# JuliaSmoothOptimizers/CaNNOLeS.jl

Measured on AMD Instinct MI355X. Metric: Newton systems/sec (fp64), batched n=1e4 NLS; achieved HBM GB/s vs peak, higher is better.
Workload: dtype f64; 1 GPU; cfg3 band constrained NLS n=10000 nequ=10000 ncon=50, 16384 independent problems per GPU, one newton_system! per problem per step; batch_per_gpu=16384, total_problems=16384, ordering=canonical+early, nnzL_stored=145150, nnzL_exact=100180, fronts=1000, all_success=True

## Files before the change

cannoles.jl_amd/csrc/band.hip:

```cpp
#include <hip/hip_runtime.h>

#include "band.h"
#include "kernels.h"

namespace cnl {

namespace {

template <class T>
__device__ __forceinline__ T* as_global(T* p) {
  return (T*)(__attribute__((address_space(1))) T*)p;
}

typedef const __attribute__((address_space(4))) int* cptr;
__device__ __forceinline__ cptr as_const(const int* p) { return (cptr)(const __attribute__((address_space(1))) int*)p; }

constexpr int NPC = BAND_NPIECE;
constexpr int LANE_D = BAND_LANE_DOUBLES;
constexpr int EXCH_OFF = BAND_IN_OFF;
static_assert(48 <= BAND_NPIECE * 8, "exchange area inside the operand pieces");

__device__ __forceinline__ constexpr int sidx(int a, int b) { return a >= b ? a * (a + 1) / 2 + b : b * (b + 1) / 2 + a; }

template <class T>
__device__ __forceinline__ T rrcp(T d) {
  T r;
  if constexpr (sizeof(T) == 8) r = __builtin_amdgcn_rcp(d);
  else r = __builtin_amdgcn_rcpf(d);
  const T e = fma(-d, r, T(1));
  return fma(r, e, r);
}
template <class T>
__device__ __forceinline__ T rdiv(T w, T d, T r) {
  const T q = w * r;
  const T res = fma(-d, q, w);
  return fma(res, r, q);
}


constexpr int NS = BAND_NS;
template <class T>
struct Win {
  T S[NS * (NS + 1) / 2];
  T X[NS];
  T S55;
  T c[NS];
  T c5;
};
__device__ __forceinline__ constexpr int lslot(int PH, int k) { return (PH - BAND_HW + k + NS) % NS; }

#define LDSD(off) (*reinterpret_cast<const T*>(myb + (off)))
#define LDSW(off) (*reinterpret_cast<T*>(myb + (off)))

struct Rec { int v[BAND_SW]; };
struct RowRec { int v[BAND_RW]; };
__device__ __forceinline__ void load_rec(Rec& R, const char* recb, int o) {
  const int4* q = reinterpret_cast<const int4*>(recb + 4 * o);
#pragma unroll
  for (int k = 0; k < BAND_SW / 4; k++) { const int4 t = q[k]; R.v[4 * k] = t.x; R.v[4 * k + 1] = t.y; R.v[4 * k + 2] = t.z; R.v[4 * k + 3] = t.w; }
}
__device__ __forceinline__ void load_row(RowRec& R, const char* recb, int o) {
  const int4* q = reinterpret_cast<const int4*>(recb + 4 * o);
#pragma unroll
  for (int k = 0; k < BAND_RW / 4; k++) { const int4 t = q[k]; R.v[4 * k] = t.x; R.v[4 * k + 1] = t.y; R.v[4 * k + 2] = t.z; R.v[4 * k + 3] = t.w; }
}

template <class T>
struct FOps { T eo[15]; T rj[BAND_NB]; T rdr, rrr; };
template <class T>
__device__ __forceinline__ void fload(FOps<T>& P, const Rec& st, const RowRec& row0, const int fl, char* myb) {
#pragma unroll
  for (int q = 0; q < 15; q++) P.eo[q] = LDSD(st.v[BS_DG0 + q]);
  static_assert(BS_RX == BS_DG0 + 14, "the fifteen operands of an entering variable are consecutive words of the step block");
  P.rdr = T(1); P.rrr = T(0);
#pragma unroll
  for (int k = 0; k < BAND_NB; k++) P.rj[k] = T(0);
  if ((fl >> 8) & 255) {
#pragma unroll
    for (int k = 0; k < BAND_NB; k++) P.rj[k] = LDSD(row0.v[BR_J0 + k]);
    P.rdr = LDSD(row0.v[BR_DI]);
    P.rrr = LDSD(row0.v[BR_RR]);
  }
}

__device__ __forceinline__ long long band_il_offset(int e, int stride) { return stride ? (long long)(e >> 3) * stride + (e & 7) : (long long)e; }

template <int PH, class T>
__device__ __forceinline__ void fstep(Win<T>& W, const FOps<T>& OP, const Rec& st, const int fl, const char* recb, const int o, char* myb,
                                      const T* __restrict__ gvals, const T* __restrict__ grhs, cptr borders, long long pv, long long pr,
                                      bool has_rhs, T rho, bool ovr, T tol, int& npos, int& nzer, const int vstride = 0, const int rstride = 0) {
  constexpr int es = PH, ps = lslot(PH, 0);
  const int nrows = (fl >> 8) & 255;
  const T (&eo)[15] = OP.eo;
  const T (&rj)[BAND_NB] = OP.rj;
  const T rdr = OP.rdr, rrr = OP.rrr;
  {
    const T dg = (eo[0] + eo[1]) + eo[2];
    T rv = eo[BS_RHO - BS_DG0];
    if (!(fl & (1 << 16))) rv = ovr ? rho : rv;
    W.S[sidx(es, es)] = dg + rv;
#pragma unroll
    for (int k = 1; k <= BAND_HW; k++) W.S[sidx(es, lslot(PH, BAND_HW - k))] = eo[BS_OD - BS_DG0 + 2 * (k - 1)] + eo[BS_OD - BS_DG0 + 2 * (k - 1) + 1];
    W.X[es] = eo[BS_BC0 - BS_DG0] + eo[BS_BC1 - BS_DG0];
    W.c[es] = eo[BS_RX - BS_DG0];
  }
  for (int i = 0; i < nrows; i++) {
    T J[BAND_NB], dr, rr;
    if (i == 0) {
#pragma unroll
      for (int k = 0; k < BAND_NB; k++) J[k] = rj[k];
      dr = rdr; rr = rrr;
    } else {
      RowRec rb;
      load_row(rb, recb, o + BAND_SW + BAND_RW * i);
#pragma unroll
      for (int k = 0; k < BAND_NB; k++) J[k] = LDSD(rb.v[BR_J0 + k]);
      dr = LDSD(rb.v[BR_DI]);
      rr = LDSD(rb.v[BR_RR]);
    }
    npos += dr > tol;
    nzer += fabs(dr) <= tol;
    const T r = rrcp(dr);
    const T w = rdiv(T(-1), dr, r);
    const T tr = rr * w;
#pragma unroll
    for (int ka = 0; ka < BAND_NB; ka++) {
      const T ta = J[ka] * w;
#pragma unroll
      for (int kb = 0; kb <= ka; kb++) W.S[sidx(lslot(PH, ka), lslot(PH, kb))] = fma(ta, J[kb], W.S[sidx(lslot(PH, ka), lslot(PH, kb))]);
      W.c[lslot(PH, ka)] = fma(tr, J[ka], W.c[lslot(PH, ka)]);
    }
  }
  if (fl & BF_PIVOT_B) {
    cptr bt = borders + BAND_BW * __builtin_amdgcn_readfirstlane(st.v[BS_BORDER]);
    W.S55 += gvals[pv + band_il_offset(bt[BB_DSRC], vstride)];
    W.c5 += has_rhs ? grhs[pr + band_il_offset(bt[BB_RHS], rstride)] : T(0);
    const T d = W.S55;
    npos += d > tol;
    nzer += fabs(d) <= tol;
    const T r = rrcp(d);
    T l[BAND_NB], w[BAND_NB];
#pragma unroll
    for (int k = 0; k < BAND_NB; k++) { w[k] = W.X[lslot(PH, k)]; l[k] = rdiv(w[k], d, r); }
    const T z = rdiv(W.c5, d, r);
#pragma unroll
    for (int ka = 0; ka < BAND_NB; ka++) {
#pragma unroll
      for (int kb = 0; kb <= ka; kb++) W.S[sidx(lslot(PH, ka), lslot(PH, kb))] = fma(w[ka], -l[kb], W.S[sidx(lslot(PH, ka), lslot(PH, kb))]);
      W.c[lslot(PH, ka)] = fma(w[ka], -z, W.c[lslot(PH, ka)]);
    }
    T* lo = reinterpret_cast<T*>(myb + st.v[BS_LB]);
#pragma unroll
    for (int k = 0; k < BAND_NB; k++) lo[k] = l[k];
    lo[BAND_NB] = z;
#pragma unroll
    for (int k = 0; k < BAND_NB; k++) W.X[lslot(PH, k)] = T(0);
    W.S55 = T(0); W.c5 = T(0);
  }
  if (fl & BF_PIVOT_X) {
    const T d = W.S[sidx(ps, ps)];
    npos += d > tol;
    nzer += fabs(d) <= tol;
    const T r = rrcp(d);
    T l[BAND_NB], w[BAND_NB];
#pragma unroll
    for (int k = 1; k < BAND_NB; k++) { w[k] = W.S[sidx(lslot(PH, k), ps)]; l[k] = rdiv(w[k], d, r); }
    const T w5 = W.X[ps], l5 = rdiv(w5, d, r), z = rdiv(W.c[ps], d, r);
#pragma unroll
    for (int ka = 1; ka < BAND_NB; ka++) {
#pragma unroll
      for (int kb = 1; kb <= ka; kb++) W.S[sidx(lslot(PH, ka), lslot(PH, kb))] = fma(w[ka], -l[kb], W.S[sidx(lslot(PH, ka), lslot(PH, kb))]);
      W.X[lslot(PH, ka)] = fma(w5, -l[ka], W.X[lslot(PH, ka)]);
      W.c[lslot(PH, ka)] = fma(w[ka], -z, W.c[lslot(PH, ka)]);
    }
    W.S55 = fma(w5, -l5, W.S55);
    W.c5 = fma(w5, -z, W.c5);
    T* lo = reinterpret_cast<T*>(myb + st.v[BS_LX]);
#pragma unroll
    for (int k = 1; k < BAND_NB; k++) lo[k - 1] = l[k];
    lo[4] = l5;
    lo[5] = z;
  }
}

template <class T>
struct BOps { T lx[BAND_LREC], lb[BAND_LREC], rj[BAND_NB]; T rdr, rrr; };
template <class T>
__device__ __forceinline__ void bload(BOps<T>& P, const Rec& st, const RowRec& row0, const int fl, char* myb) {
#pragma unroll
  for (int q = 0; q < BAND_LREC; q++) { P.lx[q] = T(0); P.lb[q] = T(0); }
#pragma unroll
  for (int k = 0; k < BAND_NB; k++) P.rj[k] = T(0);
  P.rdr = T(1); P.rrr = T(0);
  if (fl & BF_PIVOT_X) {
    const T* lo = reinterpret_cast<const T*>(myb + st.v[BS_LX]);
#pragma unroll
    for (int q = 0; q < BAND_LREC; q++) P.lx[q] = lo[q];
  }
  if (fl & BF_PIVOT_B) {
    const T* lo = reinterpret_cast<const T*>(myb + st.v[BS_LB]);
#pragma unroll
    for (int q = 0; q < BAND_LREC; q++) P.lb[q] = lo[q];
  }
  if ((fl >> 8) & 255) {
#pragma unroll
    for (int k = 0; k < BAND_NB; k++) P.rj[k] = LDSD(row0.v[BR_J0 + k]);
    P.rdr = LDSD(row0.v[BR_DI]);
    P.rrr = LDSD(row0.v[BR_RR]);
  }
}
template <int PH, class T>
__device__ __forceinline__ void bstep(T (&xs)[NS + 1], const BOps<T>& OP, const Rec& st, const RowRec& row0, const int fl, const char* recb,
                                      const int o, char* myb, cptr borders, T* __restrict__ gd, long long pd, bool okme) {
  constexpr int ps = lslot(PH, 0);
  const int nrows = (fl >> 8) & 255;
  const T (&lx)[BAND_LREC] = OP.lx;
  const T (&lb)[BAND_LREC] = OP.lb;
  const T (&rj)[BAND_NB] = OP.rj;
  const T rdr = OP.rdr, rrr = OP.rrr;
  if (fl & BF_PIVOT_X) {
    T x = lx[5];
#pragma unroll
    for (int k = 1; k < BAND_NB; k++) x = fma(-lx[k - 1], xs[lslot(PH, k)], x);
    x = fma(-lx[4], xs[NS], x);
    xs[ps] = x;
    LDSW(st.v[BS_DX]) = -x;
  }
  if (fl & BF_PIVOT_B) {
    T x = lb[BAND_NB];
#pragma unroll
    for (int k = 0; k < BAND_NB; k++) x = fma(-lb[k], xs[lslot(PH, k)], x);
    xs[NS] = x;
    if (okme) gd[pd + borders[BAND_BW * __builtin_amdgcn_readfirstlane(st.v[BS_BORDER]) + BB_DOUT]] = -x;
  }
  for (int i = 0; i < nrows; i++) {
    T J[BAND_NB], dr, rr;
    int dro;
    if (i == 0) {
#pragma unroll
      for (int k = 0; k < BAND_NB; k++) J[k] = rj[k];
      dr = rdr; rr = rrr; dro = row0.v[BR_DR];
    } else {
      RowRec rb;
      load_row(rb, recb, o + BAND_SW + BAND_RW * i);
#pragma unroll
      for (int k = 0; k < BAND_NB; k++) J[k] = LDSD(rb.v[BR_J0 + k]);
      dr = LDSD(rb.v[BR_DI]); rr = LDSD(rb.v[BR_RR]); dro = rb.v[BR_DR];
    }
    T acc = -rr;
#pragma unroll
    for (int k = 0; k < BAND_NB; k++) acc = fma(J[k], xs[lslot(PH, k)], acc);
    LDSW(dro) = rdiv(acc, dr, rrcp(dr));
  }
  if (fl & BF_ENTER_B) xs[NS] = T(0);
}

}

template <class T, int NL>
__global__ void __launch_bounds__(128, (NL <= 8 ? 2 : 1)) band_newton_kernel(const BandDev P, const LaunchArgs Ain) {
  constexpr int NI = NL / 8;
  constexpr int ES = (int)sizeof(T), LS = ES == 8 ? 3 : 2;
  static_assert(ES == 8 || ES == 4, "double or float");
  extern __shared__ double lds[];
  const int mode = Ain.mode, batch = Ain.batch;
  T* const gvals = as_global(reinterpret_cast<T*>(Ain.vals));
  const T* const grhs = as_global(reinterpret_cast<const T*>(Ain.rhs));
  T* const gd = as_global(reinterpret_cast<T*>(Ain.d));
  T* const gL = as_global(reinterpret_cast<T*>(Ain.L));
  const int lane = threadIdx.x & 63;
  const int part = __builtin_amdgcn_readfirstlane((int)(threadIdx.x >> 6));
  const int lq = lane >> 3, le = lane & 7;
  const int prob0 = blockIdx.x * NL;
  const bool has_rhs = mode != MODE_FACTOR && grhs != nullptr;
  T* const ldsT = reinterpret_cast<T*>(lds);
  char* wblk = reinterpret_cast<char*>(ldsT + (size_t)part * NL * LANE_D);
  char* recb = reinterpret_cast<char*>(ldsT + (size_t)P.nparts * NL * LANE_D) + (size_t)part * BAND_REC_MAX * 4;
  double* ctrl = reinterpret_cast<double*>(reinterpret_cast<char*>(ldsT + (size_t)P.nparts * NL * LANE_D) + (size_t)P.nparts * BAND_REC_MAX * 4);
  const int* fops_g = as_global(P.fops[part]);
  const int* bops_g = as_global(P.bops[part]);
  cptr epochs = as_const(P.epochs[part]);
  cptr borders = as_const(P.borders[part]);
  const int nepochs = P.nepochs[part];
  const int nnz = P.nnz, N = P.N;
  const long long lsize = P.lsize;
  constexpr int G8 = BAND_IL_GROUP * 8;
  static_assert(BAND_IL_GROUP % NL == 0, "a workgroup's problems lie in one group of the interleaved layout");
  const bool vil = (Ain.layout & 1) != 0, ril = (Ain.layout & 2) != 0;
  const int vstride = vil ? G8 : 0, rstride = ril ? G8 : 0;
  const long long ilg = prob0 / BAND_IL_GROUP;
  const int ilp = (prob0 % BAND_IL_GROUP) * 8;
  const T* vbase = gvals + (vil ? ilg * band_il_blocks(nnz) * G8 + ilp : (long long)prob0 * nnz);
  const T* rbase = !has_rhs ? gvals : grhs + (ril ? ilg * band_il_blocks(N) * G8 + ilp : (long long)prob0 * N);
  constexpr bool LINT = NL >= 32;
  T* lbase_g = gL + (long long)prob0 * lsize + (LINT ? 0 : P.loff[part]);
  const int loff8 = LINT ? (int)P.loff[part] : 0;
  T* dbase = gd ? gd + (long long)prob0 * N : nullptr;
  unsigned movp[NI], ldsb[NI];
  bool movok[NI];
#pragma unroll
  for (int i = 0; i < NI; i++) {
    int pl = i * 8 + lq;
    movok[i] = prob0 + pl < batch;
    if (!movok[i]) pl = batch - 1 - prob0;
    movp[i] = (unsigned)pl;
    ldsb[i] = ((unsigned)(i * 8 + lq) * (unsigned)LANE_D + (unsigned)le) << LS;
  }
  const bool clane = lane < NL;
  const int cprob = prob0 + (clane ? lane : 0);
  const bool valid = clane && cprob < batch;
  const int cpl = valid ? cprob - prob0 : batch - 1 - prob0;
  char* myb = wblk + (size_t)(clane ? lane : 0) * LANE_D * ES;
  const long long pv = vil ? ilg * band_il_blocks(nnz) * G8 + ilp + cpl * 8 : (long long)(prob0 + cpl) * nnz;
  const long long pr = ril ? ilg * band_il_blocks(N) * G8 + ilp + cpl * 8 : (long long)(prob0 + cpl) * N;
  for (int t = lane; t < NL; t += 64) *reinterpret_cast<T*>(wblk + ((size_t)t * LANE_D + BAND_ZERO_OFF) * ES) = T(0);

  const T tol = (T)Ain.params[0], kdec = (T)Ain.params[2], kinc = (T)Ain.params[3], klarge = (T)Ain.params[4], rho0 = (T)Ain.params[5],
          rhomax = (T)Ain.params[6], rhomin = (T)Ain.params[7];
  T rho = T(0), wrote = T(0);
  T rho_old = (mode == MODE_NEWTON && valid) ? as_global(reinterpret_cast<T*>(Ain.rho_old))[cprob] : T(0);
  int nfact = 0;
  bool done = !valid, success = false, ovr = false;

  static_assert(NI <= 4, "at most four problem groups per mover lane");
  T stg[NPC][NI];
  int4 rstg0;
  int pcs[NPC];
  static_assert(BAND_REC_MAX <= 256, "record buffer: one dwordx4 per lane");
#define BAND_ISSUE1(K, I) if constexpr (I < NI) stg[K][I] = *reinterpret_cast<const T*>(pb + ((movp[I] * strd + tl) << LS));
#define BAND_COMMIT1(K, I) if constexpr (I < NI) *reinterpret_cast<T*>(wblk + ldsb[I] + (BAND_IN_OFF + 8 * K) * ES) = stg[K][I];
#define BAND_ISSUE(K)                                                                                                         \
  if (pcs[K] >= 0) {                                                                                      \
    const int pc = pcs[K];                                                                                                    \
    const int arr = pc >> 28;                                                                                                 \
    const int el_ = (pc & ((1 << 28) - 1)) + (arr == 2 ? loff8 : 0);                                                          \
                    \
    const bool il_ = arr == 0 ? vil : arr == 1 ? ril : LINT;                                              \
    const int ilw_ = arr == 2 ? NL * 8 : BAND_IL_GROUP * 8;     \
    const int m_ = il_ ? (el_ & 7) : 0;                                                                                       \
    const unsigned gap_ = il_ ? (unsigned)(ilw_ - 8) : 0u;                                                                    \
    const char* pb = (arr == 0 ? reinterpret_cast<const char*>(vbase) : arr == 1 ? reinterpret_cast<const char*>(rbase)       \
                                                                                 : reinterpret_cast<const char*>(lbase_g)) +   \
                     ((il_ ? (long long)(el_ >> 3) * ilw_ : (long long)el_) << LS);                                           \
    const unsigned strd = il_ ? 8u : arr == 0 ? (unsigned)nnz : arr == 1 ? (unsigned)N : (unsigned)lsize;                     \
    const unsigned t_ = (unsigned)m_ + (unsigned)le;                                                                          \
    const unsigned tl = t_ + (t_ >> 3) * gap_;                                                                                \
    BAND_ISSUE1(K, 0) BAND_ISSUE1(K, 1) BAND_ISSUE1(K, 2) BAND_ISSUE1(K, 3)                                                   \
  }
#define BAND_COMMIT(K) { BAND_COMMIT1(K, 0) BAND_COMMIT1(K, 1) BAND_COMMIT1(K, 2) BAND_COMMIT1(K, 3) }
#define BAND_ISSUE_DESC(EP, OFS) { cptr E_ = (EP) + (OFS); _Pragma("unroll") for (int k_ = 0; k_ < NPC; k_++) pcs[k_] = E_[k_]; }
#define BAND_ISSUE_REC(OPS, OPOFF) { rstg0 = (reinterpret_cast<const int4*>((OPS) + (OPOFF)) + lane)[0]; }
#define BAND_ISSUE_ALL(EP, OFS, OPS, OPOFF)                                                                                   \
  {                                                                                                                           \
    BAND_ISSUE_DESC(EP, OFS)                                                                                                  \
    BAND_ISSUE(0) BAND_ISSUE(1) BAND_ISSUE(2) BAND_ISSUE(3) BAND_ISSUE(4) BAND_ISSUE(5) BAND_ISSUE(6) BAND_ISSUE(7)           \
    BAND_ISSUE(8) BAND_ISSUE(9) BAND_ISSUE(10) BAND_ISSUE(11) BAND_ISSUE(12) BAND_ISSUE(13) BAND_ISSUE(14)                    \
    BAND_ISSUE_REC(OPS, OPOFF)                                                                                                \
  }
#define BAND_COMMIT_ALL()                                                                                                     \
  {                                                                                                                           \
    BAND_COMMIT(0) BAND_COMMIT(1) BAND_COMMIT(2) BAND_COMMIT(3) BAND_COMMIT(4) BAND_COMMIT(5) BAND_COMMIT(6) BAND_COMMIT(7)   \
    BAND_COMMIT(8) BAND_COMMIT(9) BAND_COMMIT(10) BAND_COMMIT(11) BAND_COMMIT(12) BAND_COMMIT(13) BAND_COMMIT(14)             \
    reinterpret_cast<int4*>(recb)[lane] = rstg0;                                                                              \
  }
  static_assert(NPC == 15, "fifteen operand pieces");

  Win<T> W;
  int npos = 0, nzer = 0;
  T lj[6], zj[4];
  for (int q = 0; q < 6; q++) lj[q] = T(0);
  for (int q = 0; q < 4; q++) zj[q] = T(0);
  while (true) {
#pragma unroll
    for (int q = 0; q < NS * (NS + 1) / 2; q++) W.S[q] = T(0);
#pragma unroll
    for (int q = 0; q < NS; q++) { W.X[q] = T(0); W.c[q] = T(0); }
    W.S55 = T(0); W.c5 = T(0);
    npos = 0; nzer = 0;
    BAND_ISSUE_ALL(epochs, BE_FP, fops_g, 0)
    for (int e = 0; e < nepochs; e++) {
      cptr E = epochs + e * BAND_EW;
      BAND_COMMIT_ALL()
      const bool more_ = e + 1 < nepochs;
      if (more_) BAND_ISSUE_DESC(epochs + (e + 1) * BAND_EW, BE_FP)
      const int nst = E[BE_NSTEP];
      int o = 0;
      Rec stC, stN;
      RowRec rwC, rwN;
      load_rec(stC, recb, 0);
      load_row(rwC, recb, BAND_SW);
#define BAND_FSTEP(PHV)                                                                                                     \
      if (PHV < nst) {                                                                                                      \
        const int fl = __builtin_amdgcn_readfirstlane(stC.v[BS_FLAGS]);                                                     \
        const int onext = o + BAND_SW + BAND_RW * ((fl >> 8) & 255);                                                        \
        if (PHV + 1 < nst) { load_rec(stN, recb, onext); load_row(rwN, recb, onext + BAND_SW); }                            \
        if (clane) {                                                                                                        \
          FOps<T> op_;                                                                                                      \
          fload(op_, stC, rwC, fl, myb);                                                                                    \
          fstep<PHV>(W, op_, stC, fl, recb, o, myb, gvals, grhs, borders, pv, pr, has_rhs, rho, ovr, tol, npos, nzer, vstride, rstride); \
        }                                                                                                                   \
        o = onext; stC = stN; rwC = rwN;                                                                                    \
      }
#define BAND_LFLUSH(LB, LC)                                                                                                 \
      if (mode != MODE_FACTOR) {                                                                                            \
        const int lc_ = (LC);                                                                                               \
        const int lb_ = (LB) + loff8;                                                                                       \
        char* lout = reinterpret_cast<char*>(lbase_g) + ((LINT ? (long long)(lb_ >> 3) * (NL * 8) : (long long)lb_) << LS); \
        const unsigned t_ = (LINT ? (unsigned)(lb_ & 7) : 0u) + (unsigned)le;                                               \
        const unsigned tl = t_ + (LINT ? (t_ >> 3) * (unsigned)(NL * 8 - 8) : 0u);                                          \
        const unsigned lstr_ = LINT ? 8u : (unsigned)lsize;                                                                 \
        constexpr int lcp_ = LINT ? NL * 8 * ES : 8 * ES;                                                                   \
        T lx_[BAND_LOUT_MAX / 8][NI];                                                                                       \
        _Pragma("unroll") for (int cpc = 0; cpc < BAND_LOUT_MAX / 8; cpc++)                                                 \
          _Pragma("unroll") for (int i = 0; i < NI; i++) lx_[cpc][i] = *reinterpret_cast<const T*>(wblk + ldsb[i] + (BAND_LOUT_OFF + 8 * cpc) * ES); \
        _Pragma("unroll") for (int cpc = 0; cpc < BAND_LOUT_MAX / 8; cpc++)                                                 \
          _Pragma("unroll") for (int i = 0; i < NI; i++)                                                                    \
            if (movok[i] && cpc * 8 + le < lc_)                                                                             \
              *reinterpret_cast<T*>(lout + (((movp[i] * lstr_ + tl) << LS) + lcp_ * cpc)) = lx_[cpc][i];                     \
      }
      BAND_FSTEP(0)
      if (more_) { BAND_ISSUE(0) BAND_ISSUE(1) BAND_ISSUE(2) BAND_ISSUE(3) }
      BAND_FSTEP(1)
      if (more_) { BAND_ISSUE(4) BAND_ISSUE(5) BAND_ISSUE(6) BAND_ISSUE(7) }
      BAND_FSTEP(2)
      if (more_) { BAND_ISSUE(8) BAND_ISSUE(9) BAND_ISSUE(10) BAND_ISSUE(11) }
      BAND_FSTEP(3)
      if (more_) { BAND_ISSUE(12) BAND_ISSUE(13) BAND_ISSUE(14) BAND_ISSUE_REC(fops_g, epochs[(e + 1) * BAND_EW + BE_FOFF]) }
      BAND_LFLUSH(E[BE_LBASE], E[BE_LCNT])
      BAND_FSTEP(4) BAND_FSTEP(5) BAND_FSTEP(6) BAND_FSTEP(7)
      static_assert(BAND_EPOCH == 8, "eight step instantiations per epoch");
      if (nst == BAND_EPOCH) {
#pragma unroll
        for (int a = 0; a < NS; a++)
#pragma unroll
          for (int b = 0; b <= a; b++)
            if (b < 4) W.S[sidx(a, b)] = T(0);
#pragma unroll
        for (int a = 0; a < 4; a++) { W.X[a] = T(0); W.c[a] = T(0); }
      }
      BAND_LFLUSH(E[BE_LBASE2], E[BE_LCNT2])
    }
    int tpos = npos, tzer = nzer;
    if (P.nparts == 2) {
      if (clane) {
        T* ex = reinterpret_cast<T*>(myb + EXCH_OFF * ES);
#pragma unroll
        for (int q = 0; q < NS * (NS + 1) / 2; q++) ex[q] = W.S[q];
#pragma unroll
        for (int q = 0; q < NS; q++) ex[36 + q] = W.c[q];
        ex[44] = (T)npos; ex[45] = (T)nzer;
      }
      __syncthreads();
      if (part == 0 && clane) {
        const T* exL = reinterpret_cast<const T*>(myb + EXCH_OFF * ES);
        const T* exR = reinterpret_cast<const T*>(myb + (size_t)NL * LANE_D * ES + EXCH_OFF * ES);
        const int tL = P.m0 % NS, tR = (P.n - 1 - P.m0) % NS;
        T SJ[10], cJ[4];
#pragma unroll
        for (int i = 0; i < 4; i++) {
          const int aL = (tL + i) % NS, aR = (tR - i + NS) % NS;
#pragma unroll
          for (int j = 0; j <= i; j++) {
            const int bL = (tL + j) % NS, bR = (tR - j + NS) % NS;
            const int iL = aL >= bL ? aL * (aL + 1) / 2 + bL : bL * (bL + 1) / 2 + aL;
            const int iR = aR >= bR ? aR * (aR + 1) / 2 + bR : bR * (bR + 1) / 2 + aR;
            SJ[i * (i + 1) / 2 + j] = exL[iL] + exR[iR];
          }
          cJ[i] = exL[36 + aL] + exR[36 + aR];
        }
        tpos += (int)exR[44]; tzer += (int)exR[45];
#pragma unroll
        for (int i = 0; i < 4; i++) {
          const T d = SJ[sidx(i, i)];
          tpos += d > tol;
          tzer += fabs(d) <= tol;
          const T r = rrcp(d);
          zj[i] = rdiv(cJ[i], d, r);
          T w[4];
#pragma unroll
          for (int a = i + 1; a < 4; a++) { w[a] = SJ[sidx(a, i)]; lj[sidx(a - 1, i)] = rdiv(w[a], d, r); }
#pragma unroll
          for (int a = i + 1; a < 4; a++) {
#pragma unroll
            for (int b = i + 1; b <= a; b++) SJ[sidx(a, b)] = fma(w[a], -lj[sidx(b - 1, i)], SJ[sidx(a, b)]);
            cJ[a] = fma(w[a], -zj[i], cJ[a]);
          }
        }
      }
    }
    bool alldone = true;
    if (part == 0) {
      const bool ok = tpos == P.nvar && tzer == 0;
      if (mode == MODE_FACTOR) {
        if (valid) {
          as_global(Ain.success)[cprob] = ok ? 1 : 0;
          if (Ain.npos) as_global(Ain.npos)[cprob] = tpos;
          if (Ain.nzero) as_global(Ain.nzero)[cprob] = tzer;
        }
        done = true;
      } else if (mode == MODE_SOLVE) {
        success = ok;
        done = true;
      } else if (!done) {
        nfact++;
        if (ok) { done = true; success = true; }
        else if (nfact == 1) {
          rho = rho_old == T(0) ? rho0 : fmax(rhomin, kdec * rho_old);
          ovr = true; wrote = rho;
        } else if (rho <= rhomax) {
          rho = rho_old == T(0) ? klarge * rho : kinc * rho;
          if (rho <= rhomax) wrote = rho; else done = true;
        } else done = true;
      }
      alldone = __all(done || !clane);
      if (clane) { ctrl[lane] = rho; ctrl[NL + lane] = (ovr ? 1.0 : 0.0) + (success ? 2.0 : 0.0); }
      if (lane == 0) ctrl[2 * NL] = alldone ? 1.0 : 0.0;
    }
    if (P.nparts == 2) {
      __syncthreads();
      if (part == 1) {
        if (clane) { rho = (T)ctrl[lane]; const int f = (int)ctrl[NL + lane]; ovr = f & 1; success = f & 2; }
        alldone = ctrl[2 * NL] != 0.0;
      }
      __syncthreads();
    }
    if (alldone) break;
  }
  if (mode == MODE_FACTOR) {
    if (mode == MODE_NEWTON && part == 0 && valid) as_global(Ain.success)[cprob] = 1;
    return;
  }
  {
    T xs[NS + 1];
#pragma unroll
    for (int q = 0; q < NS + 1; q++) xs[q] = T(0);
    if (P.nparts == 2) {
      if (part == 0 && clane) {
        T xj[4];
        xj[3] = zj[3];
        xj[2] = fma(-lj[sidx(2, 2)], xj[3], zj[2]);
        xj[1] = fma(-lj[sidx(2, 1)], xj[3], fma(-lj[sidx(1, 1)], xj[2], zj[1]));
        xj[0] = fma(-lj[sidx(2, 0)], xj[3], fma(-lj[sidx(1, 0)], xj[2], fma(-lj[sidx(0, 0)], xj[1], zj[0])));
        T* ex = reinterpret_cast<T*>(myb + EXCH_OFF * ES);
        T* exR = reinterpret_cast<T*>(myb + (size_t)NL * LANE_D * ES + EXCH_OFF * ES);
#pragma unroll
        for (int i = 0; i < 4; i++) {
          ex[i] = xj[i]; exR[i] = xj[i];
          if (valid && success) gd[(long long)cprob * N + P.m0 + i] = -xj[i];
        }
      }
      __syncthreads();
      if (clane) {
        const T* ex = reinterpret_cast<const T*>(myb + EXCH_OFF * ES);
        const int t0 = part == 0 ? P.m0 % NS : (P.n - 1 - P.m0) % NS;
#pragma unroll
        for (int s = 0; s < NS; s++) {
          const int i = part == 0 ? (s - t0 + NS) % NS : (t0 - s + NS) % NS;
          xs[s] = i < 4 ? ex[i] : T(0);
        }
      }
    }
    if (part == 0 && clane) ctrl[NL + lane] = (valid && success) ? 2.0 : 0.0;
    __syncthreads();
    bool movst[NI];
#pragma unroll
    for (int i = 0; i < NI; i++) movst[i] = movok[i] && ctrl[NL + i * 8 + lq] != 0.0;
    const bool okme = valid && ctrl[NL + lane % NL] != 0.0 && clane;
    const long long pd = (long long)(prob0 + cpl) * N;
    BAND_ISSUE_ALL(epochs + (nepochs - 1) * BAND_EW, BE_BP, bops_g, 0)
    for (int e = nepochs - 1; e >= 0; e--) {
      cptr E = epochs + e * BAND_EW;
      BAND_COMMIT_ALL()
      const bool more_ = e > 0;
      if (more_) BAND_ISSUE_DESC(epochs + (e - 1) * BAND_EW, BE_BP)
      const int nst = E[BE_NSTEP];
      int o = 0;
      Rec stC, stN;
      RowRec rwC, rwN;
      load_rec(stC, recb, 0);
      load_row(rwC, recb, BAND_SW);
#define BAND_BSTEP(PHV)                                                                                                     \
      if (PHV < nst) {                                                                                                      \
        const int fl = __builtin_amdgcn_readfirstlane(stC.v[BS_FLAGS]);                                                     \
        const int onext = o + BAND_SW + BAND_RW * ((fl >> 8) & 255);                                                        \
        if (PHV > 0) { load_rec(stN, recb, onext); load_row(rwN, recb, onext + BAND_SW); }                                  \
        if (clane) {                                                                                                        \
          BOps<T> op_;                                                                                                      \
          bload(op_, stC, rwC, fl, myb);                                                                                    \
          bstep<PHV>(xs, op_, stC, rwC, fl, recb, o, myb, borders, gd, pd, okme);                                           \
        }                                                                                                                   \
        o = onext; stC = stN; rwC = rwN;                                                                                    \
      }
      BAND_BSTEP(7)
      if (more_) { BAND_ISSUE(0) BAND_ISSUE(1) BAND_ISSUE(2) BAND_ISSUE(3) }
      BAND_BSTEP(6)
      if (more_) { BAND_ISSUE(4) BAND_ISSUE(5) BAND_ISSUE(6) BAND_ISSUE(7) }
      BAND_BSTEP(5)
      if (more_) { BAND_ISSUE(8) BAND_ISSUE(9) BAND_ISSUE(10) BAND_ISSUE(11) }
      BAND_BSTEP(4)
      if (more_) { BAND_ISSUE(12) BAND_ISSUE(13) BAND_ISSUE(14) BAND_ISSUE_REC(bops_g, epochs[(e - 1) * BAND_EW + BE_BOFF]) }
      BAND_BSTEP(3) BAND_BSTEP(2) BAND_BSTEP(1) BAND_BSTEP(0)
      const int xlo = E[BE_DXLO], xc = E[BE_DXCNT], rlo = E[BE_DRLO], rc = E[BE_DRCNT];
      char* dxo = reinterpret_cast<char*>(dbase) + ((long long)xlo << LS);
      char* dro = reinterpret_cast<char*>(dbase) + ((long long)rlo << LS);
      {
        T dx_[NI], dr_[BAND_DR_MAX / 8][NI];
#pragma unroll
        for (int i = 0; i < NI; i++) dx_[i] = *reinterpret_cast<const T*>(wblk + ldsb[i] + BAND_DX_OFF * ES);
#pragma unroll
        for (int cpc = 0; cpc < BAND_DR_MAX / 8; cpc++)
#pragma unroll
          for (int i = 0; i < NI; i++) dr_[cpc][i] = *reinterpret_cast<const T*>(wblk + ldsb[i] + (BAND_DR_OFF + 8 * cpc) * ES);
#pragma unroll
        for (int i = 0; i < NI; i++)
          if (movst[i] && le < xc) *reinterpret_cast<T*>(dxo + ((movp[i] * (unsigned)N + (unsigned)le) << LS)) = dx_[i];
#pragma unroll
        for (int cpc = 0; cpc < BAND_DR_MAX / 8; cpc++)
#pragma unroll
          for (int i = 0; i < NI; i++)
            if (movst[i] && cpc * 8 + le < rc) *reinterpret_cast<T*>(dro + (((movp[i] * (unsigned)N + (unsigned)le) << LS) + 8 * ES * cpc)) = dr_[cpc][i];
      }
    }
  }
  if (part == 0 && mode == MODE_NEWTON) {
    if (nfact > 1 && rho <= rhomax) rho_old = rho;
    if (valid) {
      as_global(reinterpret_cast<T*>(Ain.rho))[cprob] = rho;
      as_global(reinterpret_cast<T*>(Ain.rho_old))[cprob] = rho_old;
      as_global(Ain.nfact)[cprob] = nfact;
      as_global(Ain.success)[cprob] = success ? 1 : 0;
    }
    for (int q = 0; q < NL; q++) {
      const int nf = __builtin_amdgcn_readlane(nfact, q);
      const int vq = __builtin_amdgcn_readlane((int)valid, q);
      if (nf > 1 && vq) {
        T wq;
        if constexpr (ES == 8) wq = __hiloint2double(__builtin_amdgcn_readlane(__double2hiint(wrote), q), __builtin_amdgcn_readlane(__double2loint(wrote), q));
        else wq = __int_as_float(__builtin_amdgcn_readlane(__float_as_int(wrote), q));
        if (vil) {
          T* vg = gvals + ilg * band_il_blocks(nnz) * G8 + ilp + q * 8;
          for (int i = lane; i < P.nvar; i += 64) vg[band_il_offset(nnz - P.nvar + i, vstride)] = wq;
        } else {
          T* vt = gvals + (long long)(prob0 + q) * nnz + (nnz - P.nvar);
          for (int i = lane; i < P.nvar; i += 64) vt[i] = wq;
        }
      }
    }
  }
}

size_t band_lds_bytes(int nparts, int nl, int esz) {
  return (size_t)nparts * nl * LANE_D * esz + (2 * (size_t)nl + 8) * sizeof(double) + (size_t)nparts * BAND_REC_MAX * 4;
}

template <class T>
static hipError_t launch_band_t(const BandDev& P, int nl, const LaunchArgs& a, hipStream_t stream) {
  const size_t ldsb = band_lds_bytes(P.nparts, nl, (int)sizeof(T));
  const int grid = (a.batch + nl - 1) / nl;
  auto go = [&](auto kern) {
    hipError_t e = hipFuncSetAttribute(reinterpret_cast<const void*>(kern), hipFuncAttributeMaxDynamicSharedMemorySize, lds_attr_cap((int)ldsb));
    if (e != hipSuccess) return e;
    hipLaunchKernelGGL(kern, dim3(grid), dim3(64 * P.nparts), ldsb, stream, P, a);
    return hipGetLastError();
  };
  if (nl == 32) return go(band_newton_kernel<T, 32>);
  if (nl == 16) return go(band_newton_kernel<T, 16>);
  if (nl == 8) return go(band_newton_kernel<T, 8>);
  return hipErrorInvalidConfiguration;
}

hipError_t launch_band(const BandDev& P, int nl, const LaunchArgs& a, hipStream_t stream) { return launch_band_t<double>(P, nl, a, stream); }
hipError_t launch_band_f32(const BandDev& P, int nl, const LaunchArgs& a, hipStream_t stream) { return launch_band_t<float>(P, nl, a, stream); }

}
```

Before: 1.487 million systems/s.

## Store factor records directly from compute lanes to global L in lane-interleaved layout

When the workgroup covers at least 32 problems, each compute lane now writes its pivot records (l coefficients and z) straight to global memory in a layout interleaved by problem, with stride NL. This replaces staging the records in LDS and flushing them later through the mover lanes. The solve-phase loads of those records are adjusted to read the new layout. The aim is to drop the LDS round trip and the flush pass, at the cost of scattered per-lane global stores issued from inside the compute step.

```diff
diff --git a/cannoles.jl_amd/csrc/band.hip b/cannoles.jl_amd/csrc/band.hip
--- a/cannoles.jl_amd/csrc/band.hip
+++ b/cannoles.jl_amd/csrc/band.hip
@@ -85,10 +85,17 @@
 
 __device__ __forceinline__ long long band_il_offset(int e, int stride) { return stride ? (long long)(e >> 3) * stride + (e & 7) : (long long)e; }
 
-template <int PH, class T>
+__host__ __device__ constexpr bool direct_records(int nl) { return nl >= 32; }
+template <class T>
+__device__ __forceinline__ int frec_index(int lds_off, int recb0) {
+  return (lds_off >> (sizeof(T) == 8 ? 3 : 2)) + recb0;
+}
+
+template <int PH, int RNL, class T>
 __device__ __forceinline__ void fstep(Win<T>& W, const FOps<T>& OP, const Rec& st, const int fl, const char* recb, const int o, char* myb,
                                       const T* __restrict__ gvals, const T* __restrict__ grhs, cptr borders, long long pv, long long pr,
-                                      bool has_rhs, T rho, bool ovr, T tol, int& npos, int& nzer, const int vstride = 0, const int rstride = 0) {
+                                      bool has_rhs, T rho, bool ovr, T tol, int& npos, int& nzer, const int vstride, const int rstride,
+                                      T* recp, const int recb0, const bool recst) {
   constexpr int es = PH, ps = lslot(PH, 0);
   const int nrows = (fl >> 8) & 255;
   const T (&eo)[15] = OP.eo;
@@ -149,10 +156,19 @@
       for (int kb = 0; kb <= ka; kb++) W.S[sidx(lslot(PH, ka), lslot(PH, kb))] = fma(w[ka], -l[kb], W.S[sidx(lslot(PH, ka), lslot(PH, kb))]);
       W.c[lslot(PH, ka)] = fma(w[ka], -z, W.c[lslot(PH, ka)]);
     }
-    T* lo = reinterpret_cast<T*>(myb + st.v[BS_LB]);
-#pragma unroll
-    for (int k = 0; k < BAND_NB; k++) lo[k] = l[k];
-    lo[BAND_NB] = z;
+    if constexpr (direct_records(RNL)) {
+      if (recst) {
+        T* lo = recp + frec_index<T>(st.v[BS_LB], recb0) * RNL;
+#pragma unroll
+        for (int k = 0; k < BAND_NB; k++) lo[k * RNL] = l[k];
+        lo[BAND_NB * RNL] = z;
+      }
+    } else {
+      T* lo = reinterpret_cast<T*>(myb + st.v[BS_LB]);
+#pragma unroll
+      for (int k = 0; k < BAND_NB; k++) lo[k] = l[k];
+      lo[BAND_NB] = z;
+    }
 #pragma unroll
     for (int k = 0; k < BAND_NB; k++) W.X[lslot(PH, k)] = T(0);
     W.S55 = T(0); W.c5 = T(0);
@@ -175,11 +191,21 @@
     }
     W.S55 = fma(w5, -l5, W.S55);
     W.c5 = fma(w5, -z, W.c5);
-    T* lo = reinterpret_cast<T*>(myb + st.v[BS_LX]);
-#pragma unroll
-    for (int k = 1; k < BAND_NB; k++) lo[k - 1] = l[k];
-    lo[4] = l5;
-    lo[5] = z;
+    if constexpr (direct_records(RNL)) {
+      if (recst) {
+        T* lo = recp + frec_index<T>(st.v[BS_LX], recb0) * RNL;
+#pragma unroll
+        for (int k = 1; k < BAND_NB; k++) lo[(k - 1) * RNL] = l[k];
+        lo[4 * RNL] = l5;
+        lo[5 * RNL] = z;
+      }
+    } else {
+      T* lo = reinterpret_cast<T*>(myb + st.v[BS_LX]);
+#pragma unroll
+      for (int k = 1; k < BAND_NB; k++) lo[k - 1] = l[k];
+      lo[4] = l5;
+      lo[5] = z;
+    }
   }
 }
 
@@ -292,9 +318,10 @@
   const int ilp = (prob0 % BAND_IL_GROUP) * 8;
   const T* vbase = gvals + (vil ? ilg * band_il_blocks(nnz) * G8 + ilp : (long long)prob0 * nnz);
   const T* rbase = !has_rhs ? gvals : grhs + (ril ? ilg * band_il_blocks(N) * G8 + ilp : (long long)prob0 * N);
-  constexpr bool LINT = NL >= 32;
-  T* lbase_g = gL + (long long)prob0 * lsize + (LINT ? 0 : P.loff[part]);
-  const int loff8 = LINT ? (int)P.loff[part] : 0;
+  constexpr bool DREC = direct_records(NL);
+  T* lbase_g = gL + (long long)prob0 * lsize + (DREC ? 0 : P.loff[part]);
+  const int loff8 = DREC ? (int)P.loff[part] : 0;
+  T* const recp = lbase_g + (long long)loff8 * NL + (lane < NL ? lane : 0);
   T* dbase = gd ? gd + (long long)prob0 * N : nullptr;
   unsigned movp[NI], ldsb[NI];
   bool movok[NI];
@@ -321,6 +348,7 @@
   T rho_old = (mode == MODE_NEWTON && valid) ? as_global(reinterpret_cast<T*>(Ain.rho_old))[cprob] : T(0);
   int nfact = 0;
   bool done = !valid, success = false, ovr = false;
+  const bool recst = valid && mode != MODE_FACTOR;
 
   static_assert(NI <= 4, "at most four problem groups per mover lane");
   T stg[NPC][NI];
@@ -334,17 +362,19 @@
     const int pc = pcs[K];                                                                                                    \
     const int arr = pc >> 28;                                                                                                 \
     const int el_ = (pc & ((1 << 28) - 1)) + (arr == 2 ? loff8 : 0);                                                          \
-                    \
-    const bool il_ = arr == 0 ? vil : arr == 1 ? ril : LINT;                                              \
+                               \
+    const bool il_ = arr == 0 ? vil : arr == 1 ? ril : DREC;                                              \
     const int ilw_ = arr == 2 ? NL * 8 : BAND_IL_GROUP * 8;     \
     const int m_ = il_ ? (el_ & 7) : 0;                                                                                       \
-    const unsigned gap_ = il_ ? (unsigned)(ilw_ - 8) : 0u;                                                                    \
+    const unsigned gap_ = il_ && !(DREC && arr == 2) ? (unsigned)(ilw_ - 8) : 0u;                                              \
+    const unsigned tm_ = arr == 2 && DREC ? (unsigned)NL : 1u;                                                                \
     const char* pb = (arr == 0 ? reinterpret_cast<const char*>(vbase) : arr == 1 ? reinterpret_cast<const char*>(rbase)       \
                                                                                  : reinterpret_cast<const char*>(lbase_g)) +   \
                      ((il_ ? (long long)(el_ >> 3) * ilw_ : (long long)el_) << LS);                                           \
-    const unsigned strd = il_ ? 8u : arr == 0 ? (unsigned)nnz : arr == 1 ? (unsigned)N : (unsigned)lsize;                     \
+    const unsigned strd = DREC ? (arr == 2 ? 1u : il_ ? 8u : arr == 0 ? (unsigned)nnz : (unsigned)N)                         \
+                               : (il_ ? 8u : arr == 0 ? (unsigned)nnz : arr == 1 ? (unsigned)N : (unsigned)lsize);             \
     const unsigned t_ = (unsigned)m_ + (unsigned)le;                                                                          \
-    const unsigned tl = t_ + (t_ >> 3) * gap_;                                                                                \
+    const unsigned tl = t_ * tm_ + (t_ >> 3) * gap_;                                                                          \
     BAND_ISSUE1(K, 0) BAND_ISSUE1(K, 1) BAND_ISSUE1(K, 2) BAND_ISSUE1(K, 3)                                                   \
   }
 #define BAND_COMMIT(K) { BAND_COMMIT1(K, 0) BAND_COMMIT1(K, 1) BAND_COMMIT1(K, 2) BAND_COMMIT1(K, 3) }
@@ -384,6 +414,7 @@
       const bool more_ = e + 1 < nepochs;
       if (more_) BAND_ISSUE_DESC(epochs + (e + 1) * BAND_EW, BE_FP)
       const int nst = E[BE_NSTEP];
+      const int recb1 = E[BE_LBASE] - BAND_LOUT_OFF, recb2 = E[BE_LBASE2] - BAND_LOUT_OFF;
       int o = 0;
       Rec stC, stN;
       RowRec rwC, rwN;
@@ -397,26 +428,24 @@
         if (clane) {                                                                                                        \
           FOps<T> op_;                                                                                                      \
           fload(op_, stC, rwC, fl, myb);                                                                                    \
-          fstep<PHV>(W, op_, stC, fl, recb, o, myb, gvals, grhs, borders, pv, pr, has_rhs, rho, ovr, tol, npos, nzer, vstride, rstride); \
+          fstep<PHV, NL>(W, op_, stC, fl, recb, o, myb, gvals, grhs, borders, pv, pr, has_rhs, rho, ovr, tol, npos, nzer, vstride, rstride, \
+                         recp, PHV < BAND_EPOCH / 2 ? recb1 : recb2, recst);                                              \
         }                                                                                                                   \
         o = onext; stC = stN; rwC = rwN;                                                                                    \
       }
 #define BAND_LFLUSH(LB, LC)                                                                                                 \
-      if (mode != MODE_FACTOR) {                                                                                            \
-        const int lc_ = (LC);                                                                                               \
-        const int lb_ = (LB) + loff8;                                                                                       \
-        char* lout = reinterpret_cast<char*>(lbase_g) + ((LINT ? (long long)(lb_ >> 3) * (NL * 8) : (long long)lb_) << LS); \
-        const unsigned t_ = (LINT ? (unsigned)(lb_ & 7) : 0u) + (unsigned)le;                                               \
-        const unsigned tl = t_ + (LINT ? (t_ >> 3) * (unsigned)(NL * 8 - 8) : 0u);                                          \
-        const unsigned lstr_ = LINT ? 8u : (unsigned)lsize;                                                                 \
-        constexpr int lcp_ = LINT ? NL * 8 * ES : 8 * ES;                                                                   \
-        T lx_[BAND_LOUT_MAX / 8][NI];                                                                                       \
-        _Pragma("unroll") for (int cpc = 0; cpc < BAND_LOUT_MAX / 8; cpc++)                                                 \
-          _Pragma("unroll") for (int i = 0; i < NI; i++) lx_[cpc][i] = *reinterpret_cast<const T*>(wblk + ldsb[i] + (BAND_LOUT_OFF + 8 * cpc) * ES); \
-        _Pragma("unroll") for (int cpc = 0; cpc < BAND_LOUT_MAX / 8; cpc++)                                                 \
-          _Pragma("unroll") for (int i = 0; i < NI; i++)                                                                    \
-            if (movok[i] && cpc * 8 + le < lc_)                                                                             \
-              *reinterpret_cast<T*>(lout + (((movp[i] * lstr_ + tl) << LS) + lcp_ * cpc)) = lx_[cpc][i];                     \
+      if constexpr (!DREC) {                                                                                                \
+        if (mode != MODE_FACTOR) {                                                                                          \
+          const int lc_ = (LC);                                                                                             \
+          char* lout = reinterpret_cast<char*>(lbase_g) + ((long long)(LB) << LS);                                          \
+          T lx_[BAND_LOUT_MAX / 8][NI];                                                                                     \
+          _Pragma("unroll") for (int cpc = 0; cpc < BAND_LOUT_MAX / 8; cpc++)                                               \
+            _Pragma("unroll") for (int i = 0; i < NI; i++) lx_[cpc][i] = *reinterpret_cast<const T*>(wblk + ldsb[i] + (BAND_LOUT_OFF + 8 * cpc) * ES); \
+          _Pragma("unroll") for (int cpc = 0; cpc < BAND_LOUT_MAX / 8; cpc++)                                               \
+            _Pragma("unroll") for (int i = 0; i < NI; i++)                                                                  \
+              if (movok[i] && cpc * 8 + le < lc_)                                                                           \
+                *reinterpret_cast<T*>(lout + (((movp[i] * (unsigned)lsize + (unsigned)le) << LS) + 8 * ES * cpc)) = lx_[cpc][i]; \
+        }                                                                                                                   \
       }
       BAND_FSTEP(0)
       if (more_) { BAND_ISSUE(0) BAND_ISSUE(1) BAND_ISSUE(2) BAND_ISSUE(3) }
```

Result: faster. 1.565 million systems/s, median of 6 (+5.3%).
